# szaguldo-kamaz/FRI-ReinforcementLearning-C

Measured on AMD Instinct MI355X. Metric: rule-distance evals/sec (rules x envs), higher is better.
Workload: dtype f64

## Files before the change

### fri-reinforcementlearning-c_amd/__init__.py

```python
import ctypes as C
import os

PKG_DIR = os.path.dirname(os.path.abspath(__file__))
ROOT = os.path.dirname(PKG_DIR)
HIP_LIB_PATH = os.environ.get("FRIRL_HIP_LIB_OVERRIDE") or os.path.join(PKG_DIR, "lib", "libfrirl_hip.so")

NO_HIT = 0xFFFFFFFF
MAX_NANT = 16
MAX_ACTIONS = 32


class FrirlHipError(RuntimeError):
    pass


class Tables(C.Structure):
    _fields_ = [("nant", C.c_int32), ("U", C.c_int32), ("u", C.c_void_p), ("ve", C.c_void_p)]


class RuleBases(C.Structure):
    _fields_ = [("E", C.c_int32), ("maxR", C.c_int32), ("rb", C.c_void_p), ("nrules", C.c_void_p), ("uidx", C.c_void_p)]


MAX_GRID = 64
# ... 17 lines not shown


class RolloutDesc(C.Structure):
    _fields_ = [("start_states", C.c_void_p), ("exclude_mask", C.c_void_p), ("rule_slot", C.c_void_p), ("steps", C.c_void_p),
                ("reward", C.c_void_p), ("success", C.c_void_p), ("final_states", C.c_void_p)]


class SenderDesc(C.Structure):
    _fields_ = [("rant", C.c_void_p), ("rule_stride", C.c_int64), ("dim_stride", C.c_int64), ("rconc", C.c_void_p), ("S", C.c_int32),
                ("reserved", C.c_int32), ("S_dev", C.c_void_p)]


class ReduceResult(C.Structure):
    _fields_ = [("rules_before", C.c_int32), ("rules_after", C.c_int32), ("rounds", C.c_int32), ("rollouts", C.c_int32),
                ("steps_incremental", C.c_int32), ("reserved", C.c_int32), ("reward", C.c_double)]


class AgentIO(C.Structure):
    _fields_ = [("obs", C.c_void_p), ("q_obs", C.c_void_p), ("reward", C.c_void_p), ("success", C.c_void_p), ("reset", C.c_void_p),
                ("action_out", C.c_void_p), ("action_idx", C.c_void_p)]


class PolicyRowsDesc(C.Structure):
    _fields_ = [("Q", C.c_int32), ("done", C.c_void_p), ("ep_steps", C.c_void_p), ("success", C.c_void_p), ("ep_reward", C.c_void_p),
                ("exclude_mask", C.c_void_p), ("rule_slot", C.c_void_p)]


class ConvergenceDesc(C.Structure):
    _fields_ = [("prev_nrules", C.c_void_p), ("prev_steps", C.c_void_p), ("prev_reward", C.c_void_p), ("prev_rconc", C.c_void_p),
                ("converged", C.c_void_p), ("episodes", C.c_void_p), ("epended", C.c_void_p)]
# ... 8 lines not shown
    "frirl_hip_last_error": (C.c_char_p, []),
    "frirl_hip_device_count": (C.c_int, []),
    "frirl_hip_device_info": (C.c_int, [C.c_int, C.c_char_p, C.c_int, C.POINTER(C.c_int32), C.POINTER(C.c_int64)]),
    "frirl_hip_set_option": (C.c_int, [C.c_char_p, C.c_int]),
    "frirl_hip_get_option": (C.c_int, [C.c_char_p, C.POINTER(C.c_int)]),
    "five_hip_rule_distance_uses_uidx": (C.c_int, [C.c_int32, C.c_int32]),
    "frirl_hip_step_uses_uidx": (C.c_int, [C.c_int32, C.c_int32, C.c_int32, C.c_int32]),
    "five_hip_rule_distance": (C.c_int, [C.POINTER(Tables), C.POINTER(RuleBases), C.c_void_p, C.c_void_p, C.c_void_p, C.c_void_p]),
    "five_hip_rule_distance_packed_words": (C.c_int, [C.c_int32, C.c_int32]),
    "frirl_hip_pack_indices": (C.c_int, [C.POINTER(Tables), C.POINTER(RuleBases), C.c_void_p, C.c_void_p]),
    "five_hip_rule_distance_packed": (C.c_int, [C.POINTER(Tables), C.POINTER(RuleBases), C.c_void_p, C.c_void_p, C.c_void_p, C.c_void_p,
                                                C.c_void_p]),
    "five_hip_rule_distance_packed_workspace_bytes": (C.c_size_t, [C.c_int32, C.c_int32, C.c_int32]),
    "five_hip_rule_distance_packed_ws": (C.c_int, [C.POINTER(Tables), C.POINTER(RuleBases), C.c_void_p, C.c_void_p, C.c_void_p, C.c_void_p,
                                                   C.c_void_p, C.c_size_t, C.c_void_p]),
    "five_hip_sqrt_unscaled_check": (C.c_int, [C.c_void_p, C.c_void_p, C.c_void_p, C.c_int64, C.c_void_p]),
    "five_hip_rule_distance_sq_guard": (C.c_int, [C.POINTER(Tables), C.c_int32, C.c_void_p, C.c_void_p, C.c_void_p]),
    "five_hip_vag_concl": (C.c_int, [C.POINTER(Tables), C.POINTER(RuleBases), C.c_int, C.c_void_p, C.c_void_p, C.c_void_p, C.c_void_p]),
    "five_hip_vag_concl_weight": (C.c_int, [C.POINTER(Tables), C.POINTER(RuleBases), C.c_int, C.c_void_p, C.c_void_p, C.c_void_p, C.c_void_p]),
    "frirl_hip_get_best_action": (C.c_int, [C.POINTER(Tables), C.POINTER(RuleBases), C.c_int, C.c_void_p, C.c_void_p, C.c_int,
                                            C.c_void_p, C.c_void_p, C.c_void_p]),
    "five_hip_vag_concl_shared": (C.c_int, [C.POINTER(Tables), C.POINTER(RuleBases), C.c_int, C.c_int32, C.c_void_p, C.c_void_p, C.c_void_p, C.c_void_p]),
    "frirl_hip_get_best_action_shared": (C.c_int, [C.POINTER(Tables), C.POINTER(RuleBases), C.c_int, C.c_int32, C.c_void_p, C.c_void_p, C.c_int,
                                                   C.c_void_p, C.c_void_p, C.c_void_p]),
    "frirl_hip_rollout_shared": (C.c_int, [C.POINTER(Tables), C.POINTER(RuleBases), C.POINTER(AgentDesc), C.c_int32, C.POINTER(RolloutDesc), C.c_void_p]),
    "frirl_hip_reduce_shared": (C.c_int, [C.POINTER(Tables), C.POINTER(RuleBases), C.POINTER(AgentDesc), C.c_void_p, C.c_int, C.c_double, C.c_int,
                                          C.POINTER(C.c_int32), C.POINTER(ReduceResult), C.c_void_p]),
    "frirl_hip_lanes_preferred": (C.c_int, [C.c_int32, C.c_int32, C.c_int32]),
    "frirl_hip_lanes_workspace_bytes": (C.c_size_t, [C.c_int32, C.c_int32, C.c_int32, C.c_int32]),
    "frirl_hip_episode_run_lanes": (C.c_int, [C.POINTER(Tables), C.POINTER(RuleBases), C.POINTER(AgentDesc), C.POINTER(EnvsDesc), C.c_int32,
# ... 132 lines not shown
        assert u.is_cuda and ve.is_cuda and rb.is_cuda and nrules.is_cuda
        assert u.dtype == torch.float64 and ve.dtype == torch.float64 and rb.dtype == torch.float64 and nrules.dtype == torch.int32
        self.nant, self.U = u.shape
        self.E, cols, self.maxR = rb.shape
        assert cols == self.nant + 1 and ve.shape == u.shape and nrules.shape == (self.E,)
        self.u, self.ve, self.rb, self.nrules = u.contiguous(), ve.contiguous(), rb.contiguous(), nrules.contiguous()
        self.uidx = None
        if uidx is not None:
            assert uidx.is_cuda and uidx.dtype == torch.int16 and uidx.shape == (self.E, self.nant, self.maxR) and self.U <= 32767
            self.uidx = uidx.contiguous()
        self.tables = Tables(self.nant, self.U, self.u.data_ptr(), self.ve.data_ptr())
        self._bases = RuleBases(self.E, self.maxR, self.rb.data_ptr(), self.nrules.data_ptr(),
                                self.uidx.data_ptr() if self.uidx is not None else None)
        self.pidx = None
        self._pidx_key = None
        W = lib().five_hip_rule_distance_packed_words(self.nant, self.U) if self.uidx is not None else 0
        if W > 0:
            self.pidx = torch.empty((self.E, W, self.maxR), dtype=torch.int32, device=self.uidx.device)
            self._pack(None)
        self._rd_ws = {}

    @property
    def bases(self):
        self._pidx_key = None
        return self._bases

    def _pack(self, stream):
        check(lib().frirl_hip_pack_indices(C.byref(self.tables), C.byref(self._bases), _ptr(self.pidx), _stream(stream)),
              "frirl_hip_pack_indices")
        self._pidx_key = (self.uidx.data_ptr(), self.uidx._version)

    def _pidx_current(self, stream):
        if self._pidx_key != (self.uidx.data_ptr(), self.uidx._version):
            self._pack(stream)
        return self.pidx

    def _rd_workspace(self, stream):
        import torch
        key = _stream(stream).value
        if key not in self._rd_ws:
            n = lib().five_hip_rule_distance_packed_workspace_bytes(self.nant, self.U, self.E)
            self._rd_ws[key] = torch.empty((n,), dtype=torch.uint8, device=self.pidx.device) if n else None
        return self._rd_ws[key]

    def rule_distance(self, x, ruledists=None, hit=None, materialise=True, stream=None):
        import torch
        assert x.is_cuda and x.dtype == torch.float64 and x.shape == (self.E, self.nant) and x.is_contiguous()
        if materialise and ruledists is None:
            ruledists = torch.empty((self.E, self.maxR), dtype=torch.float64, device=x.device)
        if hit is None:
            hit = torch.empty((self.E,), dtype=torch.int32, device=x.device)
        if self.pidx is not None:
            ws = self._rd_workspace(stream)
            rc = lib().five_hip_rule_distance_packed_ws(C.byref(self.tables), C.byref(self._bases), _ptr(self._pidx_current(stream)), _ptr(x),
                                                        _ptr(ruledists) if materialise else None, _ptr(hit), _ptr(ws),
                                                        ws.numel() if ws is not None else 0, _stream(stream))
            check(rc, "five_hip_rule_distance_packed_ws")
        else:
            rc = lib().five_hip_rule_distance(C.byref(self.tables), C.byref(self._bases), _ptr(x),
                                              _ptr(ruledists) if materialise else None, _ptr(hit), _stream(stream))
            check(rc, "five_hip_rule_distance")
        return (ruledists if materialise else None), hit

    def vag_concl(self, x, p=0, stream=None):
        import torch
        assert x.is_cuda and x.dtype == torch.float64 and x.shape == (self.E, self.nant) and x.is_contiguous()
        conc = torch.empty((self.E,), dtype=torch.float64, device=x.device)
        hit = torch.empty((self.E,), dtype=torch.int32, device=x.device)
        check(lib().five_hip_vag_concl(C.byref(self.tables), C.byref(self._bases), p, _ptr(x), _ptr(conc), _ptr(hit), _stream(stream)),
# ... 604 lines not shown
```

### fri-reinforcementlearning-c_amd/csrc/device_common.h

```cpp
#pragma once

#include <hip/hip_runtime.h>
#include <stdint.h>

#include "../../include/frirl_hip.h"

#define FRIRL_WAVE 64
#define FRIRL_BLOCK 256
#define FRIRL_WAVES_PER_BLOCK (FRIRL_BLOCK / FRIRL_WAVE)

namespace frirl {

__device__ __forceinline__ unsigned snap_index(const double *__restrict__ uni, int len, double point, double div)
{
    const int low = (int)((point - uni[0]) / div);
    if (low < 0) return 0u;
    if (low >= len) return (unsigned)(len - 1);
    if (low + 1 >= len) return (unsigned)low;
    const double d1 = uni[low] - point;
    const double d2 = uni[low + 1] - point;
    return (fabs(d1) <= fabs(d2)) ? (unsigned)low : (unsigned)(low + 1);
}

__device__ __forceinline__ double universe_div(const double *__restrict__ uni, int U)
// ... 107 lines not shown
    DeviceGuard(const DeviceGuard &) = delete;
    DeviceGuard &operator=(const DeviceGuard &) = delete;
};

struct Options {
    int no_uidx;
    int rd_unroll;
    int rd_chunk;
    int rd_nt;
    int rd_persist;
    int rd_order;
    int rd_packed;
    int rd_sqdiff;
    int rd_qpass;
    int rd_prepass;
    int step_wave;
    int step_track;
    int lanes_slices;
    int lanes_wpe;
    int rollout_group;
    int rollout_slices;
    int rollout_resident;
    int rollout_cap;
    int rollout_pair;
    int rollout_wps;
    int policy_group;
    int policy_slices;
    int learn_slices;
    int learn_alone;
    int learn_persistent;
// ... 7 lines not shown
```

### fri-reinforcementlearning-c_amd/csrc/five_rule_distance.hip

```cpp
#include <stdlib.h>

#include <type_traits>

#include "device_common.h"

namespace frirl {

__device__ __forceinline__ void item_to_env_chunk(unsigned item, int cpe, int E, bool env_fastest, int &e, int &c)
{
    if (env_fastest) { c = (int)(item / (unsigned)E); e = (int)(item - (unsigned)c * (unsigned)E); }
    else { e = (int)(item / (unsigned)cpe); c = (int)(item - (unsigned)e * (unsigned)cpe); }
}

template <int NANT, bool WRITE, int UNROLL, int NT>
__global__ __launch_bounds__(FRIRL_BLOCK) void rule_distance_kernel(
    const double *__restrict__ u, const double *__restrict__ ve, int U, const double *__restrict__ rb,
    const int32_t *__restrict__ nrules, int maxR, const double *__restrict__ x, double *__restrict__ dists,
    uint32_t *__restrict__ hit, int rules_per_block, int cpe, int E, int env_fastest)
{
    int e, c;
    item_to_env_chunk(blockIdx.x, cpe, E, env_fastest != 0, e, c);
    const int R = nrules[e];
    const int r0 = c * rules_per_block;
    if (r0 >= R) return;
// ... 400 lines not shown
                                                                   uint32_t *__restrict__ pidx)
{
    constexpr int FPW = Packed<BITS>::FPW;
    const int W = (nant + FPW - 1) / FPW;
    for (long i = (long)blockIdx.x * FRIRL_BLOCK + threadIdx.x; i < total; i += (long)gridDim.x * FRIRL_BLOCK) {
        const long e = i / maxR;
        const long r = i - e * maxR;
        const uint16_t *__restrict__ src = uidx + (size_t)e * nant * maxR + r;
        uint32_t *__restrict__ dst = pidx + (size_t)e * W * maxR + r;
        for (int w = 0; w < W; w++) {
            uint32_t v = 0u;
            for (int f = 0; f < FPW && w * FPW + f < nant; f++)
                v |= ((uint32_t)src[(size_t)(w * FPW + f) * maxR] & ((1u << BITS) - 1u)) << (BITS * f);
            dst[(size_t)w * maxR] = v;
        }
    }
}

__global__ void observe_reset_kernel(const double *__restrict__ u, const double *__restrict__ ve, int U, int nant, int E, const double *__restrict__ x,
                                     double *__restrict__ qv, uint32_t *__restrict__ hit, unsigned *__restrict__ counter)
{
    const int i = blockIdx.x * blockDim.x + threadIdx.x;
    if (i == 0) *counter = 0u;
    if (i >= E * nant) return;
    const int e = i / nant, k = i - e * nant;
    qv[i] = observe_ve(u, ve, U, k, x[i]);
    if (k == 0) hit[e] = FRIRL_HIP_NO_HIT;
}

template <int NANT, bool WRITE, int UNROLL, int BLOCK, int KB>
// ... 315 lines not shown
    } else if (hipMemsetAsync(hit, 0xFF, sizeof(uint32_t) * (size_t)b->E, s) != hipSuccess) {
        return check_launch("five_hip_rule_distance_packed(memset)");
    }
    if constexpr (NANT <= 5) {
        if (un == 4) launch_pk_form<NANT, 4>(t, b, pidx, x, qv, ruledists, hit, s, g, sq);
        else if (un == 2) launch_pk_form<NANT, 2>(t, b, pidx, x, qv, ruledists, hit, s, g, sq);
        else if (un == 1) launch_pk_form<NANT, 1>(t, b, pidx, x, qv, ruledists, hit, s, g, sq);
        else launch_pk_form<NANT, RdPkConfig<NANT>::UNROLL>(t, b, pidx, x, qv, ruledists, hit, s, g, sq);
    } else {
        launch_pk_form<NANT, RdPkConfig<NANT>::UNROLL>(t, b, pidx, x, qv, ruledists, hit, s, g, sq);
    }
    if (scratch && hipFreeAsync(scratch, s) != hipSuccess) { set_error("five_hip_rule_distance_packed: hipFreeAsync failed"); return FRIRL_HIP_ELAUNCH; }
    return check_launch("five_hip_rule_distance_packed");
}

__global__ void sqrt_unscaled_check_kernel(const double *__restrict__ a, double *__restrict__ fast, double *__restrict__ ref, long n)
{
    const long i = (long)blockIdx.x * blockDim.x + threadIdx.x;
    if (i >= n) return;
    fast[i] = sqrt_unscaled(a[i]);
    ref[i] = __dsqrt_rn(a[i]);
}

template <int NANT>
__global__ __launch_bounds__(FRIRL_BLOCK) void sq_guard_kernel(const double *__restrict__ u, const double *__restrict__ ve, int U,
                                                             const double *__restrict__ x, int32_t *__restrict__ ok)
{
    constexpr int TS = 1 << RD_PK_BITS;
    __shared__ double sq_s[NANT * TS];
    __shared__ double q_s[NANT];
// ... 124 lines not shown
{
    using namespace frirl_host;
    const int rc = check_rulebases(t, b);
    if (rc) return rc;
    const size_t need = frirl::packed_ws_bytes(t->nant, t->U, b->E);
    if (need) {
        if (!workspace || workspace_bytes < need) {
            set_error("five_hip_rule_distance_packed_ws: workspace of %zu B at %p, nant=%d U=%d E=%d needs %zu B "
                      "(five_hip_rule_distance_packed_workspace_bytes)", workspace_bytes, workspace, t->nant, t->U, b->E, need);
            return FRIRL_HIP_EINVAL;
        }
        if (reinterpret_cast<uintptr_t>(workspace) & 15) { set_error("five_hip_rule_distance_packed_ws: workspace must be 16-byte aligned"); return FRIRL_HIP_EINVAL; }
    }
    return rule_distance_packed(t, b, pidx, x, ruledists, hit, need ? workspace : nullptr, stream);
}
```

### fri-reinforcementlearning-c_amd/csrc/runtime.hip

```cpp
#include <stdarg.h>
#include <stdio.h>
#include <stdlib.h>
#include <string.h>

#include <mutex>

#include "device_common.h"

namespace frirl_host {

static thread_local char g_err[512] = "";

void set_error(const char *fmt, ...)
{
    va_list ap;
    va_start(ap, fmt);
    vsnprintf(g_err, sizeof g_err, fmt, ap);
    va_end(ap);
}

static Options g_opts;
static std::once_flag g_opts_once;
struct OptName { const char *name, *env; int Options::*field; int def; };
static const OptName k_opts[] = {
    {"no_uidx", "FRIRL_HIP_NO_UIDX", &Options::no_uidx, 0},
    {"rd_unroll", "FRIRL_HIP_RD_UNROLL", &Options::rd_unroll, 0},
    {"rd_chunk", "FRIRL_HIP_RD_CHUNK", &Options::rd_chunk, 0},
    {"rd_nt", "FRIRL_HIP_RD_NT", &Options::rd_nt, -1},
    {"rd_persist", "FRIRL_HIP_RD_PERSIST", &Options::rd_persist, -1},
    {"rd_order", "FRIRL_HIP_RD_ORDER", &Options::rd_order, 0},
    {"rd_packed", "FRIRL_HIP_RD_PACKED", &Options::rd_packed, 1},
    {"rd_sqdiff", "FRIRL_HIP_RD_SQDIFF", &Options::rd_sqdiff, 1},
    {"rd_qpass", "FRIRL_HIP_RD_QPASS", &Options::rd_qpass, 0},
    {"rd_prepass", "FRIRL_HIP_RD_PREPASS", &Options::rd_prepass, 1},
    {"step_wave", "FRIRL_HIP_STEP_WAVE", &Options::step_wave, -1},
    {"step_track", "FRIRL_HIP_STEP_TRACK", &Options::step_track, -1},
    {"lanes_slices", "FRIRL_HIP_LANES_SLICES", &Options::lanes_slices, 0},
    {"lanes_wpe", "FRIRL_HIP_LANES_WPE", &Options::lanes_wpe, 0},
    {"rollout_group", "FRIRL_HIP_ROLLOUT_GROUP", &Options::rollout_group, 0},
    {"rollout_slices", "FRIRL_HIP_ROLLOUT_SLICES", &Options::rollout_slices, 0},
    {"rollout_resident", "FRIRL_HIP_ROLLOUT_RESIDENT", &Options::rollout_resident, -1},
    {"rollout_cap", "FRIRL_HIP_ROLLOUT_CAP", &Options::rollout_cap, 0},
    {"rollout_pair", "FRIRL_HIP_ROLLOUT_PAIR", &Options::rollout_pair, -1},
    {"rollout_wps", "FRIRL_HIP_ROLLOUT_WPS", &Options::rollout_wps, 0},
    {"policy_group", "FRIRL_HIP_POLICY_GROUP", &Options::policy_group, 0},
    {"policy_slices", "FRIRL_HIP_POLICY_SLICES", &Options::policy_slices, 0},
    {"learn_slices", "FRIRL_HIP_LEARN_SLICES", &Options::learn_slices, 0},
    {"learn_alone", "FRIRL_HIP_LEARN_ALONE", &Options::learn_alone, 0},
    {"learn_persistent", "FRIRL_HIP_LEARN_PERSISTENT", &Options::learn_persistent, -1},
// ... 122 lines not shown
```

### include/frirl_hip.h

```cpp
#ifndef FRIRL_HIP_H
#define FRIRL_HIP_H

#include <stdint.h>

#ifdef __cplusplus
extern "C" {
#endif

#define FRIRL_HIP_MAX_NANT     16
#define FRIRL_HIP_MAX_ACTIONS  32
#define FRIRL_HIP_MAX_GRID     64
#define FRIRL_HIP_NO_HIT       0xFFFFFFFFu

#define FRIRL_HIP_ENV_MOUNTAINCAR 0
#define FRIRL_HIP_ENV_CARTPOLE    1
#define FRIRL_HIP_ENV_ACROBOT     2
#define FRIRL_HIP_ENV_EXTERNAL    3

#define FRIRL_HIP_UPD_INACTIVE   0
#define FRIRL_HIP_UPD_EXACT      1
#define FRIRL_HIP_UPD_SPREAD     2
#define FRIRL_HIP_UPD_INSERTED   3
#define FRIRL_HIP_UPD_SKIPPED    4
#define FRIRL_HIP_UPD_FULL       5
// ... 26 lines not shown
int frirl_hip_set_option(const char *name, int value);
int frirl_hip_get_option(const char *name, int *value);
int five_hip_rule_distance_uses_uidx(int32_t nant, int32_t U);
int frirl_hip_step_uses_uidx(int32_t nant, int32_t U, int32_t maxR, int32_t E);

int five_hip_rule_distance(const frirl_hip_tables *t, const frirl_hip_rulebases *b, const double *x,
                           double *ruledists, uint32_t *hit, void *stream);

int five_hip_rule_distance_packed_words(int32_t nant, int32_t U);
int frirl_hip_pack_indices(const frirl_hip_tables *t, const frirl_hip_rulebases *b, uint32_t *pidx, void *stream);
int five_hip_rule_distance_packed(const frirl_hip_tables *t, const frirl_hip_rulebases *b, const uint32_t *pidx, const double *x,
                                  double *ruledists, uint32_t *hit, void *stream);
size_t five_hip_rule_distance_packed_workspace_bytes(int32_t nant, int32_t U, int32_t E);
int five_hip_rule_distance_packed_ws(const frirl_hip_tables *t, const frirl_hip_rulebases *b, const uint32_t *pidx, const double *x,
                                     double *ruledists, uint32_t *hit, void *workspace, size_t workspace_bytes, void *stream);
int five_hip_sqrt_unscaled_check(const double *a, double *fast, double *ref, int64_t n, void *stream);
int five_hip_rule_distance_sq_guard(const frirl_hip_tables *t, int32_t E, const double *x, int32_t *ok, void *stream);

int five_hip_vag_concl(const frirl_hip_tables *t, const frirl_hip_rulebases *b, int p, const double *x,
                       double *conc, uint32_t *hit, void *stream);

int five_hip_vag_concl_weight(const frirl_hip_tables *t, const frirl_hip_rulebases *b, int p, const double *x,
                              double *weights, uint32_t *hit, void *stream);

int frirl_hip_get_best_action(const frirl_hip_tables *t, const frirl_hip_rulebases *b, int p, const double *states,
                              const double *action_ve, int A, double *actconc, int32_t *best, void *stream);

typedef struct frirl_hip_agent {
    double alpha, gamma;
    double qdiff_pos_boundary;
// ... 244 lines not shown
```

Measured before the change: 508.4 billion.

## Add 3-byte mixed-radix rule codes for rule distance with nant up to 5

Adds a compact encoding of each rule's per-antecedent universe indices. Only the indices that actually occur are ranked, and the ranks are combined into one mixed-radix code of at most 24 bits, stored as a 16-bit low part plus an 8-bit high part. The rule-distance kernel decodes these codes with multiply-high reciprocals and reads squared differences from per-env tables built from the observed values. This cuts the bytes read per rule compared with the packed-word index format. In exchange the pack step costs more (a mask scan, a device-to-host sync and a round-trip decode check) and the kernel does extra integer decode work.

```diff
diff --git a/fri-reinforcementlearning-c_amd/__init__.py b/fri-reinforcementlearning-c_amd/__init__.py
--- a/fri-reinforcementlearning-c_amd/__init__.py
+++ b/fri-reinforcementlearning-c_amd/__init__.py
@@ -55,6 +55,12 @@
 class ReduceResult(C.Structure):
     _fields_ = [("rules_before", C.c_int32), ("rules_after", C.c_int32), ("rounds", C.c_int32), ("rollouts", C.c_int32),
                 ("steps_incremental", C.c_int32), ("reserved", C.c_int32), ("reward", C.c_double)]
+
+
+class Code3Plan(C.Structure):
+    _fields_ = [("nant", C.c_int32), ("fits", C.c_int32), ("tree", C.c_uint32), ("n", C.c_uint32 * 5), ("prod", C.c_uint32 * 6),
+                ("big_d", C.c_uint32 * 2), ("big_m", C.c_uint32 * 2), ("big_t", C.c_uint32 * 2), ("pair_m", C.c_uint32 * 2),
+                ("rank_of", (C.c_uint8 * 64) * 5), ("index_of", (C.c_uint8 * 64) * 5)]
 
 
 class AgentIO(C.Structure):
@@ -93,6 +99,12 @@
     "five_hip_rule_distance_packed_workspace_bytes": (C.c_size_t, [C.c_int32, C.c_int32, C.c_int32]),
     "five_hip_rule_distance_packed_ws": (C.c_int, [C.POINTER(Tables), C.POINTER(RuleBases), C.c_void_p, C.c_void_p, C.c_void_p, C.c_void_p,
                                                    C.c_void_p, C.c_size_t, C.c_void_p]),
+    "frirl_hip_code3_masks": (C.c_int, [C.POINTER(Tables), C.POINTER(RuleBases), C.c_void_p, C.c_void_p]),
+    "frirl_hip_code3_plan_build": (C.c_int, [C.c_int32, C.POINTER(C.c_uint64), C.POINTER(Code3Plan)]),
+    "frirl_hip_code3_decode_check": (C.c_int64, [C.POINTER(Code3Plan), C.c_uint32, C.c_uint32]),
+    "frirl_hip_code3_pack": (C.c_int, [C.POINTER(Tables), C.POINTER(RuleBases), C.POINTER(Code3Plan), C.c_void_p, C.c_void_p, C.c_void_p, C.c_void_p]),
+    "five_hip_rule_distance_code3_ws": (C.c_int, [C.POINTER(Tables), C.POINTER(RuleBases), C.POINTER(Code3Plan), C.c_void_p, C.c_void_p, C.c_void_p,
+                                                  C.c_void_p, C.c_void_p, C.c_void_p, C.c_void_p, C.c_size_t, C.c_void_p]),
     "five_hip_sqrt_unscaled_check": (C.c_int, [C.c_void_p, C.c_void_p, C.c_void_p, C.c_int64, C.c_void_p]),
     "five_hip_rule_distance_sq_guard": (C.c_int, [C.POINTER(Tables), C.c_int32, C.c_void_p, C.c_void_p, C.c_void_p]),
     "five_hip_vag_concl": (C.c_int, [C.POINTER(Tables), C.POINTER(RuleBases), C.c_int, C.c_void_p, C.c_void_p, C.c_void_p, C.c_void_p]),
@@ -255,6 +267,7 @@
                                 self.uidx.data_ptr() if self.uidx is not None else None)
         self.pidx = None
         self._pidx_key = None
+        self.code3 = self.code_lo = self.code_hi = None
         W = lib().five_hip_rule_distance_packed_words(self.nant, self.U) if self.uidx is not None else 0
         if W > 0:
             self.pidx = torch.empty((self.E, W, self.maxR), dtype=torch.int32, device=self.uidx.device)
@@ -267,8 +280,32 @@
         return self._bases
 
     def _pack(self, stream):
+        import torch
         check(lib().frirl_hip_pack_indices(C.byref(self.tables), C.byref(self._bases), _ptr(self.pidx), _stream(stream)),
               "frirl_hip_pack_indices")
+        self.code3 = None
+        if self.nant <= 5:
+            s = stream if stream is not None else torch.cuda.current_stream()
+            with torch.cuda.stream(s):
+                scratch = torch.zeros((8,), dtype=torch.int64, device=self.uidx.device)
+            check(lib().frirl_hip_code3_masks(C.byref(self.tables), C.byref(self._bases), _ptr(scratch), _stream(stream)), "frirl_hip_code3_masks")
+            with torch.cuda.stream(s):
+                masks = scratch[:self.nant].cpu()
+            plan = Code3Plan()
+            host = (C.c_uint64 * self.nant)(*[int(m) & 0xFFFFFFFFFFFFFFFF for m in masks.tolist()])
+            fits = lib().frirl_hip_code3_plan_build(self.nant, host, C.byref(plan))
+            check(min(fits, 0), "frirl_hip_code3_plan_build")
+            if fits == 1:
+                if self.code_lo is None:
+                    self.code_lo = torch.empty((self.E, self.maxR), dtype=torch.int16, device=self.uidx.device)
+                    self.code_hi = torch.empty((self.E, self.maxR), dtype=torch.uint8, device=self.uidx.device)
+                bad = scratch[7:8]
+                check(lib().frirl_hip_code3_pack(C.byref(self.tables), C.byref(self._bases), C.byref(plan), _ptr(self.code_lo), _ptr(self.code_hi),
+                                                 _ptr(bad), _stream(stream)), "frirl_hip_code3_pack")
+                with torch.cuda.stream(s):
+                    if int(bad.cpu()[0]) != 0:
+                        raise FrirlHipError("frirl_hip_code3_pack: a rule's code does not decode to its ranks")
+                self.code3 = plan
         self._pidx_key = (self.uidx.data_ptr(), self.uidx._version)
 
     def _pidx_current(self, stream):
@@ -293,7 +330,14 @@
             hit = torch.empty((self.E,), dtype=torch.int32, device=x.device)
         if self.pidx is not None:
             ws = self._rd_workspace(stream)
-            rc = lib().five_hip_rule_distance_packed_ws(C.byref(self.tables), C.byref(self._bases), _ptr(self._pidx_current(stream)), _ptr(x),
+            pidx = self._pidx_current(stream)
+            if self.code3 is not None:
+                rc = lib().five_hip_rule_distance_code3_ws(C.byref(self.tables), C.byref(self._bases), C.byref(self.code3), _ptr(self.code_lo),
+                                                           _ptr(self.code_hi), _ptr(pidx), _ptr(x), _ptr(ruledists) if materialise else None,
+                                                           _ptr(hit), _ptr(ws), ws.numel() if ws is not None else 0, _stream(stream))
+                check(rc, "five_hip_rule_distance_code3_ws")
+                return (ruledists if materialise else None), hit
+            rc = lib().five_hip_rule_distance_packed_ws(C.byref(self.tables), C.byref(self._bases), _ptr(pidx), _ptr(x),
                                                         _ptr(ruledists) if materialise else None, _ptr(hit), _ptr(ws),
                                                         ws.numel() if ws is not None else 0, _stream(stream))
             check(rc, "five_hip_rule_distance_packed_ws")
diff --git a/fri-reinforcementlearning-c_amd/csrc/code3.h b/fri-reinforcementlearning-c_amd/csrc/code3.h
--- /dev/null
+++ b/fri-reinforcementlearning-c_amd/csrc/code3.h
@@ -0,0 +1,149 @@
+#pragma once
+
+#include <stdint.h>
+
+#include "../../include/frirl_hip.h"
+
+#if defined(__HIPCC__)
+#include <hip/hip_runtime.h>
+#define FRIRL_HD __host__ __device__ inline __attribute__((always_inline))
+#else
+#define FRIRL_HD inline
+#endif
+
+namespace frirl {
+
+static constexpr int C3_MAX_NANT = FRIRL_HIP_CODE3_MAX_NANT;
+static constexpr uint32_t C3_LIMIT = 1u << 24;
+static constexpr int C3_PAIR_SHIFT = 20;
+
+struct Code3Dec {
+    uint32_t tree;
+    uint32_t n[C3_MAX_NANT];
+    uint32_t prod[C3_MAX_NANT + 1];
+    uint32_t big_d[2], big_m[2], big_t[2];
+    uint32_t pair_m[2];
+};
+
+FRIRL_HD uint32_t c3_mulhi24(uint32_t a, uint32_t b)
+{
+    return (uint32_t)(((uint64_t)(a & 0xFFFFFFu) * (uint64_t)(b & 0xFFFFFFu)) >> 32);
+}
+FRIRL_HD uint32_t c3_mul24(uint32_t a, uint32_t b)
+{
+#if defined(__HIP_DEVICE_COMPILE__)
+    uint32_t r;
+    asm("v_mul_u32_u24 %0, %1, %2" : "=v"(r) : "v"(a), "s"(b));
+    return r;
+#else
+    return (a & 0xFFFFFFu) * (b & 0xFFFFFFu);
+#endif
+}
+FRIRL_HD uint32_t c3_big_div(uint32_t x, const Code3Dec &p, int i) { return c3_mulhi24(x, p.big_m[i]) >> p.big_t[i]; }
+FRIRL_HD void c3_pair(uint32_t x, uint32_t n, uint32_t m, uint32_t &lo, uint32_t &hi)
+{
+    hi = c3_mul24(x, m) >> C3_PAIR_SHIFT;
+    lo = x - c3_mul24(hi, n);
+}
+
+template <int NANT, int FORM = -1>
+FRIRL_HD void code3_decode(uint32_t code, const Code3Dec &p, uint32_t (&rank)[NANT])
+{
+    static_assert(NANT >= 1 && NANT <= C3_MAX_NANT, "code3 serves nant <= 5");
+    if (NANT == 1) { rank[0] = code; return; }
+    if (FORM == 1 || (FORM < 0 && p.tree)) {
+        if (NANT == 2) {
+            c3_pair(code, p.n[0], p.pair_m[0], rank[0], rank[NANT > 1 ? 1 : 0]);
+        } else if (NANT == 3) {
+            const uint32_t b = c3_big_div(code, p, 0);
+            const uint32_t a = code - c3_mul24(b, p.big_d[0]);
+            rank[NANT > 2 ? 2 : 0] = b;
+            c3_pair(a, p.n[0], p.pair_m[0], rank[0], rank[NANT > 1 ? 1 : 0]);
+        } else if (NANT == 4) {
+            const uint32_t b = c3_big_div(code, p, 0);
+            const uint32_t a = code - c3_mul24(b, p.big_d[0]);
+            c3_pair(a, p.n[0], p.pair_m[0], rank[0], rank[NANT > 1 ? 1 : 0]);
+            c3_pair(b, p.n[NANT > 2 ? 2 : 0], p.pair_m[1], rank[NANT > 2 ? 2 : 0], rank[NANT > 3 ? 3 : 0]);
+        } else {
+            const uint32_t b = c3_big_div(code, p, 0);
+            const uint32_t a = code - c3_mul24(b, p.big_d[0]);
+            c3_pair(b, p.n[NANT > 3 ? 3 : 0], p.pair_m[1], rank[NANT > 3 ? 3 : 0], rank[NANT > 4 ? 4 : 0]);
+            const uint32_t r2 = c3_big_div(a, p, 1);
+            const uint32_t a2 = a - c3_mul24(r2, p.big_d[1]);
+            rank[NANT > 2 ? 2 : 0] = r2;
+            c3_pair(a2, p.n[0], p.pair_m[0], rank[0], rank[NANT > 1 ? 1 : 0]);
+        }
+        return;
+    }
+#if defined(__HIPCC__)
+#pragma unroll
+#endif
+    for (int k = 0; k < NANT; k++) rank[k] = (code / p.prod[k]) % p.n[k];
+}
+
+template <int NANT>
+FRIRL_HD uint32_t code3_encode(const uint32_t (&rank)[NANT], const Code3Dec &p)
+{
+    uint32_t c = rank[0];
+#if defined(__HIPCC__)
+#pragma unroll
+#endif
+    for (int k = 1; k < NANT; k++) c += rank[k] * p.prod[k];
+    return c;
+}
+
+inline Code3Dec code3_dec_of(const frirl_hip_code3_plan &pl)
+{
+    Code3Dec d;
+    d.tree = pl.tree;
+    for (int k = 0; k < C3_MAX_NANT; k++) d.n[k] = pl.n[k];
+    for (int k = 0; k <= C3_MAX_NANT; k++) d.prod[k] = pl.prod[k];
+    for (int i = 0; i < 2; i++) { d.big_d[i] = pl.big_d[i]; d.big_m[i] = pl.big_m[i]; d.big_t[i] = pl.big_t[i]; d.pair_m[i] = pl.pair_m[i]; }
+    return d;
+}
+
+inline bool code3_big_params(uint32_t d, uint32_t xmax, uint32_t &m, uint32_t &t)
+{
+    if (d < 2) return false;
+    for (t = 0; t < 16; t++) {
+        const uint64_t two_s = 1ull << (32 + t);
+        const uint64_t mm = (two_s + d - 1) / d;
+        if (mm >= C3_LIMIT) continue;
+        const uint64_t e = mm * d - two_s;
+        if ((uint64_t)xmax * e < two_s) { m = (uint32_t)mm; return true; }
+    }
+    return false;
+}
+
+inline void code3_plan_build(int nant, const uint64_t *masks, frirl_hip_code3_plan *pl)
+{
+    *pl = frirl_hip_code3_plan{};
+    pl->nant = nant;
+    if (nant < 1 || nant > C3_MAX_NANT) return;
+    uint64_t total = 1;
+    for (int k = 0; k < C3_MAX_NANT; k++) {
+        const uint64_t mk = k < nant ? masks[k] : 1ull;
+        uint32_t n = 0;
+        for (int i = 0; i < 64; i++)
+            if (mk >> i & 1) { pl->rank_of[k][i] = (uint8_t)n; pl->index_of[k][n] = (uint8_t)i; n++; }
+        if (!n) return;
+        pl->n[k] = n;
+        pl->prod[k] = (uint32_t)total;
+        total *= n;
+        if (total > C3_LIMIT) return;
+    }
+    pl->prod[C3_MAX_NANT] = (uint32_t)total;
+    pl->fits = 1;
+    const uint32_t cmax = (uint32_t)total - 1;
+    for (int i = 0; i < 2; i++) pl->pair_m[i] = 0;
+    bool ok = true;
+    auto pair = [&](int i, int k) { pl->pair_m[i] = ((1u << C3_PAIR_SHIFT) + pl->n[k] - 1) / pl->n[k]; };
+    auto big = [&](int i, int k, uint32_t xmax) { pl->big_d[i] = pl->prod[k]; ok = ok && code3_big_params(pl->prod[k], xmax, pl->big_m[i], pl->big_t[i]); };
+    if (nant == 2) pair(0, 0);
+    else if (nant == 3) { big(0, 2, cmax); pair(0, 0); }
+    else if (nant == 4) { big(0, 2, cmax); pair(0, 0); pair(1, 2); }
+    else if (nant == 5) { big(0, 3, cmax); big(1, 2, pl->prod[3] - 1); pair(0, 0); pair(1, 3); }
+    pl->tree = ok ? 1u : 0u;
+}
+
+}
diff --git a/fri-reinforcementlearning-c_amd/csrc/device_common.h b/fri-reinforcementlearning-c_amd/csrc/device_common.h
--- a/fri-reinforcementlearning-c_amd/csrc/device_common.h
+++ b/fri-reinforcementlearning-c_amd/csrc/device_common.h
@@ -145,6 +145,7 @@
     int rd_sqdiff;
     int rd_qpass;
     int rd_prepass;
+    int rd_code3;
     int step_wave;
     int step_track;
     int lanes_slices;
diff --git a/fri-reinforcementlearning-c_amd/csrc/five_rule_distance.hip b/fri-reinforcementlearning-c_amd/csrc/five_rule_distance.hip
--- a/fri-reinforcementlearning-c_amd/csrc/five_rule_distance.hip
+++ b/fri-reinforcementlearning-c_amd/csrc/five_rule_distance.hip
@@ -3,6 +3,7 @@
 #include <type_traits>
 
 #include "device_common.h"
+#include "code3.h"
 
 namespace frirl {
 
@@ -438,6 +439,202 @@
                 v |= ((uint32_t)src[(size_t)(w * FPW + f) * maxR] & ((1u << BITS) - 1u)) << (BITS * f);
             dst[(size_t)w * maxR] = v;
         }
+    }
+}
+
+struct Code3Tab { uint32_t n[C3_MAX_NANT]; uint8_t index_of[C3_MAX_NANT][64]; };
+
+__global__ __launch_bounds__(FRIRL_BLOCK) void code3_masks_kernel(const uint16_t *__restrict__ uidx, int nant, int maxR, long total,
+                                                                  unsigned long long *__restrict__ masks)
+{
+    unsigned long long m[C3_MAX_NANT] = {};
+    for (long i = (long)blockIdx.x * FRIRL_BLOCK + threadIdx.x; i < total; i += (long)gridDim.x * FRIRL_BLOCK) {
+        const long e = i / maxR;
+        const long r = i - e * maxR;
+        const uint16_t *__restrict__ src = uidx + (size_t)e * nant * maxR + r;
+#pragma unroll
+        for (int k = 0; k < C3_MAX_NANT; k++)
+            if (k < nant) m[k] |= 1ull << (src[(size_t)k * maxR] & 63u);
+    }
+#pragma unroll
+    for (int k = 0; k < C3_MAX_NANT; k++) {
+        if (k >= nant) break;
+        unsigned lo = (unsigned)m[k], hi = (unsigned)(m[k] >> 32);
+#pragma unroll
+        for (int off = 32; off > 0; off >>= 1) {
+            lo |= (unsigned)__shfl_xor((int)lo, off, FRIRL_WAVE);
+            hi |= (unsigned)__shfl_xor((int)hi, off, FRIRL_WAVE);
+        }
+        const unsigned long long v = ((unsigned long long)hi << 32) | lo;
+        if ((threadIdx.x & (FRIRL_WAVE - 1)) == 0 && v) atomicOr(&masks[k], v);
+    }
+}
+
+struct Code3Rank { uint8_t rank_of[C3_MAX_NANT][64]; unsigned long long used[C3_MAX_NANT]; };
+
+template <int NANT>
+__global__ __launch_bounds__(FRIRL_BLOCK) void code3_pack_kernel(const uint16_t *__restrict__ uidx, int maxR, long total, Code3Dec dec, Code3Rank rk,
+                                                                 uint16_t *__restrict__ lo, uint8_t *__restrict__ hi, uint32_t *__restrict__ bad)
+{
+    for (long i = (long)blockIdx.x * FRIRL_BLOCK + threadIdx.x; i < total; i += (long)gridDim.x * FRIRL_BLOCK) {
+        const long e = i / maxR;
+        const long r = i - e * maxR;
+        const uint16_t *__restrict__ src = uidx + (size_t)e * NANT * maxR + r;
+        uint32_t rank[NANT], back[NANT];
+        bool ok = true;
+#pragma unroll
+        for (int k = 0; k < NANT; k++) {
+            const uint32_t ix = src[(size_t)k * maxR] & 63u;
+            ok = ok && (rk.used[k] >> ix & 1ull);
+            rank[k] = rk.rank_of[k][ix];
+        }
+        const uint32_t code = code3_encode<NANT>(rank, dec);
+        code3_decode<NANT>(code, dec, back);
+#pragma unroll
+        for (int k = 0; k < NANT; k++) ok = ok && back[k] == rank[k];
+        lo[i] = (uint16_t)(code & 0xFFFFu);
+        hi[i] = (uint8_t)(code >> 16);
+        if (!ok && bad) *bad = 1u;
+    }
+}
+
+template <int NANT, int BITS>
+__global__ __launch_bounds__(FRIRL_BLOCK) void sq_tables_c3_kernel(const double *__restrict__ u, const double *__restrict__ ve, int U, int E,
+                                                                 const double *__restrict__ x, Code3Tab tab, double *__restrict__ sqtab,
+                                                                 uint32_t *__restrict__ fastv, uint32_t *__restrict__ hit)
+{
+    constexpr int TS = 1 << BITS, N = NANT * TS;
+    static_assert(TS == 64, "Code3Tab rows hold 64 ranks");
+    __shared__ double q_s[FRIRL_WAVES_PER_BLOCK][NANT];
+    const int lane = threadIdx.x & (FRIRL_WAVE - 1), wave = threadIdx.x / FRIRL_WAVE;
+    const int e = blockIdx.x * FRIRL_WAVES_PER_BLOCK + wave;
+    const bool live = e < E;
+    double tv[(N + FRIRL_WAVE - 1) / FRIRL_WAVE];
+#pragma unroll
+    for (int m = 0; m < (N + FRIRL_WAVE - 1) / FRIRL_WAVE; m++) {
+        const int i = lane + m * FRIRL_WAVE;
+        const int k = i >> BITS, j = i & (TS - 1);
+        tv[m] = (i < N && (uint32_t)j < tab.n[k]) ? ve[k * U + tab.index_of[k][j]] : 0.0;
+    }
+    if (live && lane < NANT) q_s[wave][lane] = observe_ve(u, ve, U, lane, x[(size_t)e * NANT + lane]);
+    __syncthreads();
+    if (!live) return;
+    const bool ok = fill_sq_table<NANT, BITS, FRIRL_WAVE>(q_s[wave], sqtab + (size_t)e * N, tv, lane);
+    const bool fast = __all(ok);
+    if (lane == 0) {
+        fastv[e] = fast ? 1u : 0u;
+        hit[e] = FRIRL_HIP_NO_HIT;
+    }
+}
+
+template <int NANT, int BITS, bool FAST, bool TREE>
+__device__ __forceinline__ void c3_pair_sq(uint32_t lo, uint32_t hi, const Code3Dec &dec, const double *__restrict__ sq_s, double2 &d, bool &z0, bool &z1)
+{
+    constexpr int TS = 1 << BITS;
+    const uint32_t c0 = __builtin_amdgcn_perm(hi, lo, 0x0c040100u), c1 = __builtin_amdgcn_perm(hi, lo, 0x0c050302u);
+    uint32_t r0[NANT], r1[NANT];
+    code3_decode<NANT, TREE ? 1 : 0>(c0, dec, r0);
+    code3_decode<NANT, TREE ? 1 : 0>(c1, dec, r1);
+    double a0 = sq_s[r0[0]], a1 = sq_s[r1[0]];
+#pragma unroll
+    for (int k = 1; k < NANT; k++) {
+        a0 = a0 + sq_s[k * TS + r0[k]];
+        a1 = a1 + sq_s[k * TS + r1[k]];
+    }
+    if (FAST) {
+        d.x = sqrt_unscaled(a0);
+        d.y = sqrt_unscaled(a1);
+        z0 = a0 == 0.0;
+        z1 = a1 == 0.0;
+    } else {
+        d.x = __dsqrt_rn(a0);
+        d.y = __dsqrt_rn(a1);
+        z0 = d.x == 0.0;
+        z1 = d.y == 0.0;
+    }
+}
+
+template <int NANT, bool WRITE, int UNROLL, int BITS>
+__global__ __launch_bounds__(FRIRL_BLOCK) void rule_distance_c3_kernel(
+    const uint16_t *__restrict__ lo, const uint8_t *__restrict__ hi, Code3Dec dec, const int32_t *__restrict__ nrules, int maxR,
+    double *__restrict__ dists, uint32_t *__restrict__ hit, int rules_per_block, int cpe, int E, int env_fastest,
+    const double *__restrict__ sqtab, const uint32_t *__restrict__ fastv)
+{
+    constexpr int TS = 1 << BITS;
+    __shared__ __attribute__((aligned(16))) double sq_s[NANT * TS];
+    __shared__ unsigned red_s[FRIRL_WAVES_PER_BLOCK];
+    int e, c;
+    if (env_fastest == 0) {
+        const unsigned grp = blockIdx.x / (unsigned)(RD_XCDS * cpe), j = blockIdx.x - grp * (unsigned)(RD_XCDS * cpe);
+        e = (int)(grp * RD_XCDS + j % RD_XCDS);
+        c = (int)(j / RD_XCDS);
+        if (e >= E) return;
+    } else {
+        item_to_env_chunk(blockIdx.x, cpe, E, env_fastest == 1, e, c);
+    }
+    const int R = nrules[e];
+    const int r0 = c * rules_per_block;
+    if (r0 >= R) return;
+    int r_end = r0 + rules_per_block;
+    if (r_end > R) r_end = R;
+
+    const uint16_t *__restrict__ lo_e = lo + (size_t)e * maxR;
+    const uint8_t *__restrict__ hi_e = hi + (size_t)e * maxR;
+    constexpr int STEP = FRIRL_BLOCK * 2;
+    uint32_t wl[UNROLL];
+    uint16_t wh[UNROLL];
+    auto load = [&](int r) {
+#pragma unroll
+        for (int j = 0; j < UNROLL; j++) {
+            const int rr = r + j * STEP;
+            if (rr < r_end) {
+                wl[j] = __builtin_nontemporal_load(reinterpret_cast<const uint32_t *>(lo_e + rr));
+                wh[j] = __builtin_nontemporal_load(reinterpret_cast<const uint16_t *>(hi_e + rr));
+            }
+        }
+    };
+    int r = r0 + 2 * (int)threadIdx.x;
+    load(r);
+    double *__restrict__ out = WRITE ? dists + (size_t)e * maxR : nullptr;
+    unsigned best = FRIRL_HIP_NO_HIT;
+
+    constexpr int N2 = NANT * TS / 2;
+    const double2 *__restrict__ src = reinterpret_cast<const double2 *>(sqtab + (size_t)e * (NANT * TS));
+    for (int i = threadIdx.x; i < N2; i += FRIRL_BLOCK) reinterpret_cast<double2 *>(sq_s)[i] = src[i];
+    const bool fast = fastv[e] != 0u;
+    __syncthreads();
+    auto sweep = [&](auto fast_tag, auto tree_tag) {
+        constexpr bool FAST = decltype(fast_tag)::value, TREE = decltype(tree_tag)::value;
+        for (; r < r_end; r += STEP * UNROLL) {
+            if (r != r0 + 2 * (int)threadIdx.x) load(r);
+#pragma unroll
+            for (int j = 0; j < UNROLL; j++) {
+                const int rr = r + j * STEP;
+                if (rr < r_end) {
+                    double2 d;
+                    bool z0, z1;
+                    c3_pair_sq<NANT, BITS, FAST, TREE>(wl[j], (uint32_t)wh[j], dec, sq_s, d, z0, z1);
+                    if (WRITE) { __builtin_nontemporal_store(d.x, out + rr); __builtin_nontemporal_store(d.y, out + rr + 1); }
+                    if (z1 && rr + 1 < R) best = min(best, (unsigned)(rr + 1));
+                    if (z0) best = min(best, (unsigned)rr);
+                }
+            }
+        }
+    };
+    if (dec.tree) {
+        if (fast) sweep(std::true_type{}, std::true_type{});
+        else sweep(std::false_type{}, std::true_type{});
+    } else {
+        if (fast) sweep(std::true_type{}, std::false_type{});
+        else sweep(std::false_type{}, std::false_type{});
+    }
+    best = wave_min_u32(best);
+    if ((threadIdx.x & (FRIRL_WAVE - 1)) == 0) red_s[threadIdx.x / FRIRL_WAVE] = best;
+    __syncthreads();
+    if (threadIdx.x == 0) {
+        unsigned m = red_s[0];
+        for (int v = 1; v < FRIRL_WAVES_PER_BLOCK; v++) m = red_s[v] < m ? red_s[v] : m;
+        if (m != FRIRL_HIP_NO_HIT) atomicMin(&hit[e], m);
     }
 }
 
@@ -783,6 +980,48 @@
     return check_launch("five_hip_rule_distance_packed");
 }
 
+template <int NANT, int UN>
+static void launch_c3(const frirl_hip_tables *t, const frirl_hip_rulebases *b, const frirl_hip_code3_plan *pl, const uint16_t *lo, const uint8_t *hi,
+                      const double *x, double *ruledists, uint32_t *hit, void *ws, hipStream_t s, const RdGrid &g)
+{
+    double *sqtab = static_cast<double *>(ws);
+    uint32_t *fastv = reinterpret_cast<uint32_t *>(sqtab + (size_t)b->E * NANT * (1 << RD_PK_BITS));
+    const int order = frirl_host::opts().rd_order;
+    const unsigned items = order == 0 ? (unsigned)g.cpe * (unsigned)((b->E + RD_XCDS - 1) / RD_XCDS * RD_XCDS) : g.items;
+    Code3Tab tab;
+    for (int k = 0; k < C3_MAX_NANT; k++) {
+        tab.n[k] = pl->n[k];
+        for (int j = 0; j < 64; j++) tab.index_of[k][j] = pl->index_of[k][j];
+    }
+    const Code3Dec dec = code3_dec_of(*pl);
+    hipLaunchKernelGGL((sq_tables_c3_kernel<NANT, RD_PK_BITS>), dim3((unsigned)((b->E + FRIRL_WAVES_PER_BLOCK - 1) / FRIRL_WAVES_PER_BLOCK)), dim3(FRIRL_BLOCK),
+                       0, s, t->u, t->ve, t->U, b->E, x, tab, sqtab, fastv, hit);
+    if (ruledists)
+        hipLaunchKernelGGL((rule_distance_c3_kernel<NANT, true, UN, RD_PK_BITS>), dim3(items), dim3(FRIRL_BLOCK), 0, s, lo, hi, dec, b->nrules, b->maxR,
+                           ruledists, hit, g.rules_per_block, g.cpe, b->E, order, sqtab, fastv);
+    else
+        hipLaunchKernelGGL((rule_distance_c3_kernel<NANT, false, UN, RD_PK_BITS>), dim3(items), dim3(FRIRL_BLOCK), 0, s, lo, hi, dec, b->nrules, b->maxR,
+                           ruledists, hit, g.rules_per_block, g.cpe, b->E, order, sqtab, fastv);
+}
+
+template <int NANT>
+static int launch_code3(const frirl_hip_tables *t, const frirl_hip_rulebases *b, const frirl_hip_code3_plan *pl, const uint16_t *lo, const uint8_t *hi,
+                        const double *x, double *ruledists, uint32_t *hit, void *ws, hipStream_t s)
+{
+    using namespace frirl_host;
+    const RdTune tn = rd_tune();
+    const int un = tn.unroll ? tn.unroll : RdPkConfig<NANT>::UNROLL_PRE;
+    RdGrid g;
+    if (!make_grid(b, tn.chunk > 0 ? tn.chunk : 2 * FRIRL_BLOCK * un, g) || (long)g.cpe * ((long)b->E + RD_XCDS) > 0x7FFFFFFFL) {
+        set_error("five_hip_rule_distance_code3_ws: too many work items");
+        return FRIRL_HIP_EINVAL;
+    }
+    if (un == 8) launch_c3<NANT, 8>(t, b, pl, lo, hi, x, ruledists, hit, ws, s, g);
+    else if (un == 2) launch_c3<NANT, 2>(t, b, pl, lo, hi, x, ruledists, hit, ws, s, g);
+    else launch_c3<NANT, 4>(t, b, pl, lo, hi, x, ruledists, hit, ws, s, g);
+    return check_launch("five_hip_rule_distance_code3_ws");
+}
+
 __global__ void sqrt_unscaled_check_kernel(const double *__restrict__ a, double *__restrict__ fast, double *__restrict__ ref, long n)
 {
     const long i = (long)blockIdx.x * blockDim.x + threadIdx.x;
@@ -937,3 +1176,136 @@
     }
     return rule_distance_packed(t, b, pidx, x, ruledists, hit, need ? workspace : nullptr, stream);
 }
+
+static bool code3_shape(const frirl_hip_tables *t) { return frirl::packed_words(t->nant, t->U) && t->nant <= frirl::C3_MAX_NANT; }
+
+extern "C" int frirl_hip_code3_masks(const frirl_hip_tables *t, const frirl_hip_rulebases *b, uint64_t *masks, void *stream)
+{
+    using namespace frirl_host;
+    int rc = check_rulebases(t, b);
+    if (rc) return rc;
+    if (!b->uidx || !masks) { set_error("frirl_hip_code3_masks: NULL uidx/masks"); return FRIRL_HIP_EINVAL; }
+    if (!code3_shape(t)) { set_error("frirl_hip_code3_masks: nant=%d U=%d is not served by the 3-byte codes", t->nant, t->U); return FRIRL_HIP_EINVAL; }
+    if (reinterpret_cast<uintptr_t>(masks) & 7) { set_error("frirl_hip_code3_masks: masks must be 8-byte aligned"); return FRIRL_HIP_EINVAL; }
+    if ((rc = check_device())) return rc;
+    hipStream_t s = as_stream(stream);
+    if (hipMemsetAsync(masks, 0, sizeof(uint64_t) * (size_t)t->nant, s) != hipSuccess) return check_launch("frirl_hip_code3_masks(memset)");
+    const long total = (long)b->E * b->maxR;
+    long grid = (total + FRIRL_BLOCK - 1) / FRIRL_BLOCK;
+    if (grid > (long)frirl::device_cus() * 32) grid = (long)frirl::device_cus() * 32;
+    hipLaunchKernelGGL(frirl::code3_masks_kernel, dim3((unsigned)grid), dim3(FRIRL_BLOCK), 0, s, b->uidx, t->nant, b->maxR, total,
+                       reinterpret_cast<unsigned long long *>(masks));
+    return check_launch("frirl_hip_code3_masks");
+}
+
+extern "C" int frirl_hip_code3_plan_build(int32_t nant, const uint64_t *masks, frirl_hip_code3_plan *plan)
+{
+    using namespace frirl_host;
+    if (!masks || !plan) { set_error("frirl_hip_code3_plan_build: NULL masks/plan"); return FRIRL_HIP_EINVAL; }
+    if (nant < 1 || nant > FRIRL_HIP_MAX_NANT) { set_error("frirl_hip_code3_plan_build: nant=%d", nant); return FRIRL_HIP_EINVAL; }
+    frirl::code3_plan_build(nant, masks, plan);
+    return plan->fits ? 1 : 0;
+}
+
+template <int NANT>
+static int64_t code3_check(const frirl::Code3Dec &dec, uint32_t first, uint32_t end)
+{
+    for (uint32_t c = first; c < end; c++) {
+        uint32_t rank[NANT];
+        frirl::code3_decode<NANT>(c, dec, rank);
+        for (int k = 0; k < NANT; k++)
+            if (rank[k] != (c / dec.prod[k]) % dec.n[k]) return (int64_t)c;
+    }
+    return -1;
+}
+
+extern "C" int64_t frirl_hip_code3_decode_check(const frirl_hip_code3_plan *plan, uint32_t first, uint32_t count)
+{
+    if (!plan || !plan->fits || plan->nant < 1 || plan->nant > frirl::C3_MAX_NANT) return -2;
+    const uint32_t total = plan->prod[frirl::C3_MAX_NANT];
+    if (first > total || count > total - first) return -2;
+    const frirl::Code3Dec dec = frirl::code3_dec_of(*plan);
+    switch (plan->nant) {
+    case 1: return code3_check<1>(dec, first, first + count);
+    case 2: return code3_check<2>(dec, first, first + count);
+    case 3: return code3_check<3>(dec, first, first + count);
+    case 4: return code3_check<4>(dec, first, first + count);
+    default: return code3_check<5>(dec, first, first + count);
+    }
+}
+
+static int code3_plan_checked(const char *who, const frirl_hip_tables *t, const frirl_hip_code3_plan *plan)
+{
+    using namespace frirl_host;
+    if (!plan || !plan->fits || plan->nant != t->nant || plan->prod[frirl::C3_MAX_NANT] < 1 || plan->prod[frirl::C3_MAX_NANT] > frirl::C3_LIMIT) {
+        set_error("%s: the plan does not fit or is not of nant=%d", who, t->nant);
+        return FRIRL_HIP_EINVAL;
+    }
+    for (int k = 0; k < frirl::C3_MAX_NANT; k++) {
+        if (plan->n[k] < 1 || plan->n[k] > 64) { set_error("%s: plan radix %u", who, plan->n[k]); return FRIRL_HIP_EINVAL; }
+        for (uint32_t j = 0; j < plan->n[k]; j++)
+            if (k < t->nant && plan->index_of[k][j] >= t->U) { set_error("%s: plan index %d >= U=%d", who, plan->index_of[k][j], t->U); return FRIRL_HIP_EINVAL; }
+    }
+    return FRIRL_HIP_OK;
+}
+
+extern "C" int frirl_hip_code3_pack(const frirl_hip_tables *t, const frirl_hip_rulebases *b, const frirl_hip_code3_plan *plan, uint16_t *lo,
+                                    uint8_t *hi, uint32_t *bad, void *stream)
+{
+    using namespace frirl_host;
+    int rc = check_rulebases(t, b);
+    if (rc) return rc;
+    if (!b->uidx || !lo || !hi) { set_error("frirl_hip_code3_pack: NULL uidx/lo/hi"); return FRIRL_HIP_EINVAL; }
+    if (!code3_shape(t)) { set_error("frirl_hip_code3_pack: nant=%d U=%d is not served by the 3-byte codes", t->nant, t->U); return FRIRL_HIP_EINVAL; }
+    if ((rc = code3_plan_checked("frirl_hip_code3_pack", t, plan))) return rc;
+    if ((reinterpret_cast<uintptr_t>(lo) & 3) || (reinterpret_cast<uintptr_t>(hi) & 1)) { set_error("frirl_hip_code3_pack: lo must be 4-byte, hi 2-byte aligned"); return FRIRL_HIP_EINVAL; }
+    if ((rc = check_device())) return rc;
+    const long total = (long)b->E * b->maxR;
+    long grid = (total + FRIRL_BLOCK - 1) / FRIRL_BLOCK;
+    if (grid > (long)frirl::device_cus() * 32) grid = (long)frirl::device_cus() * 32;
+    const frirl::Code3Dec dec = frirl::code3_dec_of(*plan);
+    frirl::Code3Rank rk;
+    for (int k = 0; k < frirl::C3_MAX_NANT; k++) {
+        rk.used[k] = 0;
+        for (int j = 0; j < 64; j++) rk.rank_of[k][j] = plan->rank_of[k][j];
+        for (uint32_t j = 0; j < plan->n[k]; j++) rk.used[k] |= 1ull << plan->index_of[k][j];
+    }
+    switch (t->nant) {
+#define FRIRL_CASE(N) case N: hipLaunchKernelGGL(frirl::code3_pack_kernel<N>, dim3((unsigned)grid), dim3(FRIRL_BLOCK), 0, as_stream(stream), b->uidx, b->maxR, total, dec, rk, lo, hi, bad); break;
+        FRIRL_CASE(1) FRIRL_CASE(2) FRIRL_CASE(3) FRIRL_CASE(4) FRIRL_CASE(5)
+#undef FRIRL_CASE
+    }
+    return check_launch("frirl_hip_code3_pack");
+}
+
+extern "C" int five_hip_rule_distance_code3_ws(const frirl_hip_tables *t, const frirl_hip_rulebases *b, const frirl_hip_code3_plan *plan,
+                                               const uint16_t *lo, const uint8_t *hi, const uint32_t *pidx, const double *x, double *ruledists,
+                                               uint32_t *hit, void *workspace, size_t workspace_bytes, void *stream)
+{
+    using namespace frirl_host;
+    int rc = check_rulebases(t, b);
+    if (rc) return rc;
+    const Options &o = opts();
+    if (!code3_shape(t) || !plan || !plan->fits || o.rd_code3 == 0 || !o.rd_prepass || !o.rd_sqdiff || !o.rd_packed || o.no_uidx || o.rd_persist == 1)
+        return five_hip_rule_distance_packed_ws(t, b, pidx, x, ruledists, hit, workspace, workspace_bytes, stream);
+    const size_t need = frirl::packed_ws_bytes(t->nant, t->U, b->E);
+    if (!workspace || workspace_bytes < need) {
+        set_error("five_hip_rule_distance_code3_ws: workspace of %zu B at %p, nant=%d U=%d E=%d needs %zu B "
+                  "(five_hip_rule_distance_packed_workspace_bytes)", workspace_bytes, workspace, t->nant, t->U, b->E, need);
+        return FRIRL_HIP_EINVAL;
+    }
+    if (reinterpret_cast<uintptr_t>(workspace) & 15) { set_error("five_hip_rule_distance_code3_ws: workspace must be 16-byte aligned"); return FRIRL_HIP_EINVAL; }
+    if ((rc = code3_plan_checked("five_hip_rule_distance_code3_ws", t, plan))) return rc;
+    if (!lo || !hi || !x || !hit) { set_error("five_hip_rule_distance_code3_ws: NULL lo/hi/x/hit"); return FRIRL_HIP_EINVAL; }
+    if ((reinterpret_cast<uintptr_t>(lo) & 3) || (reinterpret_cast<uintptr_t>(hi) & 1)) { set_error("five_hip_rule_distance_code3_ws: lo must be 4-byte, hi 2-byte aligned"); return FRIRL_HIP_EINVAL; }
+    if (ruledists && (reinterpret_cast<uintptr_t>(ruledists) & 15)) { set_error("five_hip_rule_distance_code3_ws: ruledists must be 16-byte aligned"); return FRIRL_HIP_EINVAL; }
+    if ((rc = check_device())) return rc;
+    hipStream_t s = as_stream(stream);
+    switch (t->nant) {
+#define FRIRL_CASE(N) case N: return frirl::launch_code3<N>(t, b, plan, lo, hi, x, ruledists, hit, workspace, s);
+        FRIRL_CASE(1) FRIRL_CASE(2) FRIRL_CASE(3) FRIRL_CASE(4) FRIRL_CASE(5)
+#undef FRIRL_CASE
+    }
+    set_error("five_hip_rule_distance_code3_ws: unsupported nant=%d", t->nant);
+    return FRIRL_HIP_EINVAL;
+}
diff --git a/fri-reinforcementlearning-c_amd/csrc/runtime.hip b/fri-reinforcementlearning-c_amd/csrc/runtime.hip
--- a/fri-reinforcementlearning-c_amd/csrc/runtime.hip
+++ b/fri-reinforcementlearning-c_amd/csrc/runtime.hip
@@ -33,6 +33,7 @@
     {"rd_sqdiff", "FRIRL_HIP_RD_SQDIFF", &Options::rd_sqdiff, 1},
     {"rd_qpass", "FRIRL_HIP_RD_QPASS", &Options::rd_qpass, 0},
     {"rd_prepass", "FRIRL_HIP_RD_PREPASS", &Options::rd_prepass, 1},
+    {"rd_code3", "FRIRL_HIP_RD_CODE3", &Options::rd_code3, -1},
     {"step_wave", "FRIRL_HIP_STEP_WAVE", &Options::step_wave, -1},
     {"step_track", "FRIRL_HIP_STEP_TRACK", &Options::step_track, -1},
     {"lanes_slices", "FRIRL_HIP_LANES_SLICES", &Options::lanes_slices, 0},
diff --git a/include/frirl_hip.h b/include/frirl_hip.h
--- a/include/frirl_hip.h
+++ b/include/frirl_hip.h
@@ -64,6 +64,25 @@
 size_t five_hip_rule_distance_packed_workspace_bytes(int32_t nant, int32_t U, int32_t E);
 int five_hip_rule_distance_packed_ws(const frirl_hip_tables *t, const frirl_hip_rulebases *b, const uint32_t *pidx, const double *x,
                                      double *ruledists, uint32_t *hit, void *workspace, size_t workspace_bytes, void *stream);
+#define FRIRL_HIP_CODE3_MAX_NANT 5
+typedef struct frirl_hip_code3_plan {
+    int32_t nant;
+    int32_t fits;
+    uint32_t tree;
+    uint32_t n[FRIRL_HIP_CODE3_MAX_NANT];
+    uint32_t prod[FRIRL_HIP_CODE3_MAX_NANT + 1];
+    uint32_t big_d[2], big_m[2], big_t[2], pair_m[2];
+    uint8_t rank_of[FRIRL_HIP_CODE3_MAX_NANT][64];
+    uint8_t index_of[FRIRL_HIP_CODE3_MAX_NANT][64];
+} frirl_hip_code3_plan;
+int frirl_hip_code3_masks(const frirl_hip_tables *t, const frirl_hip_rulebases *b, uint64_t *masks, void *stream);
+int frirl_hip_code3_plan_build(int32_t nant, const uint64_t *masks, frirl_hip_code3_plan *plan);
+int64_t frirl_hip_code3_decode_check(const frirl_hip_code3_plan *plan, uint32_t first, uint32_t count);
+int frirl_hip_code3_pack(const frirl_hip_tables *t, const frirl_hip_rulebases *b, const frirl_hip_code3_plan *plan, uint16_t *lo,
+                         uint8_t *hi, uint32_t *bad, void *stream);
+int five_hip_rule_distance_code3_ws(const frirl_hip_tables *t, const frirl_hip_rulebases *b, const frirl_hip_code3_plan *plan,
+                                    const uint16_t *lo, const uint8_t *hi, const uint32_t *pidx, const double *x, double *ruledists,
+                                    uint32_t *hit, void *workspace, size_t workspace_bytes, void *stream);
 int five_hip_sqrt_unscaled_check(const double *a, double *fast, double *ref, int64_t n, void *stream);
 int five_hip_rule_distance_sq_guard(const frirl_hip_tables *t, int32_t E, const double *x, int32_t *ok, void *stream);
 
```

Result: faster. 516.4 billion (median of 6 runs) (+1.6%).
